# better62/MM-VQA-Healthcare

Measured on AMD Instinct MI355X. Metric: image-question pairs/sec, M3AE-base fine-tune step (fwd+bwd+AdamW) @384px, higher is better.
Workload: dtype bf16

## Files before the change

### include/m3ae_hip.h

```cpp
#ifndef M3AE_HIP_H
#define M3AE_HIP_H

#include <stdint.h>

#ifdef __cplusplus
extern "C" {
#endif

#define M3AE_ABI_VERSION 4

enum { M3AE_F32 = 0, M3AE_BF16 = 1 };
enum { M3AE_ACT_NONE = 0, M3AE_ACT_GELU = 1, M3AE_ACT_QUICKGELU = 2, M3AE_ACT_TANH = 3, M3AE_ACT_RELU = 4,
       M3AE_ACT_MULAUX = 5  };
enum { M3AE_ERR_ARG = -1, M3AE_ERR_UNSUPPORTED = -2, M3AE_ERR_ALIGN = -3, M3AE_ERR_WORKSPACE = -4 };

int m3ae_abi_version(void);
void m3ae_desc_sizes(int64_t out3[3]);
const char* m3ae_last_gemm_path(void);

typedef struct {
    int64_t M, N, K;
    int64_t batch1, batch2;
    const void* A; int64_t a_sm, a_sk, a_sb1, a_sb2;
    const void* B; int64_t b_sk, b_sn, b_sb1, b_sb2;
    void* C;       int64_t c_sm, c_sn, c_sb1, c_sb2;
    int32_t dtype_a, dtype_b, dtype_c;
    float alpha;
    int32_t accumulate;
    const float* bias;
    int32_t act;
    void* preact;
    const void* residual;
    const void* dact_aux;
    int32_t dact;
    int32_t force_generic;
    float* a_rowsum;
    float dropout_p;
    uint64_t dropout_seed;
    int32_t preact_grad;
    int32_t launch_flags;
    const void* dropout_salt;
} m3ae_gemm_desc;
enum { M3AE_GEMM_NO_PERSISTENT = 1 };
#define M3AE_GEMM_NT_VARIANT(v) ((((v) + 1) & 0xf) << 8)
#define M3AE_GEMM_TN_VARIANT(v) ((((v) + 1) & 0xf) << 12)
#define M3AE_GEMM_COL_GROUP(g) (((g) & 0xf) << 16)
int m3ae_gemm(const m3ae_gemm_desc* d, void* stream);

typedef struct {
    int64_t B, H, Lq, Lk, Dh;
    const void* q; int64_t q_sb, q_sl;
    const void* k; int64_t k_sb, k_sl;
    const void* v; int64_t v_sb, v_sl;
    void* o;       int64_t o_sb, o_sl;
    const float* key_mask;
    const float* pos_bias;
    float scale;
    int32_t causal;
    float* lse; int64_t lse_stride;
    int32_t dtype;
    void* workspace; int64_t workspace_bytes;
    const void* d_o;
    void* dq; void* dk; void* dv;
    float* delta;
    float* d_pos_bias;
    float dropout_p;
    uint64_t dropout_seed;
    const void* dropout_salt;
    int32_t launch_flags;
} m3ae_attn_desc;
enum { M3AE_ATTN_LEGACY_KERNELS = 1 };
int64_t m3ae_attn_workspace_bytes(const m3ae_attn_desc* d, int backward);
int m3ae_attn_fwd(const m3ae_attn_desc* d, void* stream);
int m3ae_attn_bwd(const m3ae_attn_desc* d, void* stream);
int m3ae_attn_probs(const m3ae_attn_desc* d, float* probs, int64_t p_sb, int64_t p_sh, int64_t p_sq, void* stream);

typedef struct {
    int32_t dir;
    int64_t B, Lq, Lk, D, H;
    const void* x;
    const void* y;
    const float* key_mask;
    const void *wq, *wq_t, *wkv, *wkv_t, *wo, *wo_t;
    const float *bq, *bkv, *bo, *ln_g, *ln_b;
    float ln_eps;
    float dropout_p;
    uint64_t seed_attn, seed_hidden;
    void* proj;
    void* prime;
    float* colbias;
    void* probs;
    void* probs_drop;
    float* rowsum;
    void* zctx;
    void* ctx;
    void* s;
    void* out;
    float *mean, *rstd;
    const void* d_out;
    void* dx;
    void* dy;
    float *g_wq, *g_wkv, *g_wo, *g_bq, *g_bkv, *g_bo, *g_ln_g, *g_ln_b;
    void* ws_ds;
    void* ws_dsd;
    void* ws_dscores;
    void* ws_dprime;
    void* ws_dproj;
    void* ws_dz;
    void* ws_dctx;
    float* ws_vec;
    float* ws_ln;
    int32_t launch_flags;
    const void* dropout_salt;
} m3ae_xattn_desc;
enum { M3AE_XATTN_NO_PERSISTENT = 1,
       M3AE_XATTN_LEGACY_CHAIN = 2     };
int m3ae_xattn_supported(const m3ae_xattn_desc* d);
int m3ae_xattn_bwd_supported(const m3ae_xattn_desc* d);
int64_t m3ae_xattn_probs_ld(const m3ae_xattn_desc* d);
int m3ae_xattn_fwd(const m3ae_xattn_desc* d, void* stream);
int m3ae_xattn_bwd(const m3ae_xattn_desc* d, void* stream);
int m3ae_xattn_probs_export(const m3ae_xattn_desc* d, int dropped, float* out, int64_t o_sb, int64_t o_sh, int64_t o_sq,
                            void* stream);

int m3ae_layernorm_fwd(const void* x, const float* gamma, const float* beta, void* y, float* mean, float* rstd,
                       int64_t M, int64_t D, float eps, int dtype, int act, int rms, void* stream);
int64_t m3ae_layernorm_bwd_blocks(int64_t M);
int m3ae_layernorm_bwd(const void* dy, const void* x, const float* gamma, const float* beta, const float* mean,
                       const float* rstd, void* dx, const void* dx_add, float* dgamma, float* dbeta, float* workspace,
                       int64_t M, int64_t D, int dtype, int act, int rms, void* stream);
int m3ae_layernorm_bwd_drop(const void* dy, const void* x, const float* gamma, const float* beta, const float* mean,
                            const float* rstd, void* dx, void* dx_drop, float dropout_p, uint64_t dropout_seed,
                            const void* dropout_salt, float* dgamma, float* dbeta, float* workspace, int64_t M, int64_t D,
                            int dtype, void* stream);
int m3ae_dropout(const void* x, void* out, uint8_t* keep_mask, int64_t rows, int64_t cols, float p, uint64_t seed,
                 const void* salt, int dtype, void* stream);

int m3ae_colsum(const void* x, float* out, int64_t M, int64_t N, int64_t ldx, int dtype, int accumulate,
                void* stream);

int m3ae_roberta_embed_fwd(const int64_t* ids, const float* word, const float* pos, const float* type, void* out,
                           int64_t B, int64_t S, int64_t D, int64_t pad_id, int dtype, void* stream);
int m3ae_roberta_embed_bwd(const int64_t* ids, const void* d_out, float* d_word, float* d_pos, float* d_type,
                           int64_t B, int64_t S, int64_t D, int64_t pad_id, int dtype, void* stream);

int m3ae_patchify(const float* img, void* out, int64_t B, int64_t R, int64_t P, int dtype, void* stream);
int m3ae_image_normalize_u8(const uint8_t* in, float* out, int64_t B, int64_t H, int64_t W, const float* mean3,
                            const float* std3, void* stream);
int m3ae_vit_tokens_fwd(const void* patch, const float* cls, const float* pos, void* out, int64_t B, int64_t G,
                        int64_t D, int dtype, void* stream);
int m3ae_vit_tokens_bwd(const void* d_out, void* d_patch, float* d_cls, float* d_pos, int64_t B, int64_t G,
                        int64_t D, int dtype, void* stream);

int m3ae_bce_logits(const void* logits, const float* targets, float* loss, void* d_logits, int64_t B, int64_t C,
// ... 36 lines not shown
```

### mm-vqa-healthcare_amd/csrc/attention.hip

```cpp
#include "common.h"
#include <stdlib.h>
#include <type_traits>

int m3ae_gemm_generic(const m3ae_gemm_desc& d, hipStream_t s);

namespace {

constexpr float LOG2E = 1.4426950408889634f;
constexpr int VRS = 192;
constexpr int TILE_LDS = 32 * VRS;

struct AttnArgs {
    const bf16_t* q; int64_t q_sb, q_sl;
    const bf16_t* k; int64_t k_sb, k_sl;
    const bf16_t* v; int64_t v_sb, v_sl;
    bf16_t* o; int64_t o_sb, o_sl;
    const float* key_mask;
    const float* pos_bias;
    float scale, scale_log2;
    int causal;
    float* lse; int64_t lse_stride;
    int64_t B, H, Lq, Lk;
    const bf16_t* d_o;
    bf16_t* dq; bf16_t* dk; bf16_t* dv;
// ... 214 lines not shown
    float m[NQ], l[NQ];
#pragma unroll
    for (int n = 0; n < NQ; ++n) {
        qi[n] = q0 + 32 * n + r;
        const int64_t qrow = qi[n] < a.Lq ? qi[n] : a.Lq - 1;
        const bf16_t* qp = a.q + b * a.q_sb + qrow * a.q_sl + head * 64;
#pragma unroll
        for (int ks = 0; ks < 4; ++ks) qf[n][ks] = row_frag(qp, ks, h);
        brow[n] = BIAS ? a.pos_bias + ((int64_t)head * a.Lq + qrow) * a.Lk : nullptr;
        o[n][0] = zero16(); o[n][1] = zero16();
        m[n] = -1e30f; l[n] = 0.f;
    }
    const bf16_t* kbase = a.k + b * a.k_sb + head * 64;
    const bf16_t* vbase = a.v + b * a.v_sb + head * 64;
    const float* mrow = MASK ? a.key_mask + b * a.Lk : nullptr;
    const int nkt = (int)((a.Lk + 31) / 32);

    s16x8 kreg = coop_load(kbase, a.k_sl, 0, a.Lk, t);
    s16x8 vreg = coop_load(vbase, a.v_sl, 0, a.Lk, t);
    put_row_img(lds, kreg, t);
    put_tr_img(lds + RIMG, vreg, t);
    if (nkt > 1) {
        kreg = coop_load(kbase, a.k_sl, 32, a.Lk, t);
        vreg = coop_load(vbase, a.v_sl, 32, a.Lk, t);
    }
    coop_barrier();
    for (int kt = 0; kt < nkt; ++kt) {
        const bool last = kt + 1 == nkt;
        s16x8 kreg2 = kreg, vreg2 = vreg;
        if (kt + 2 < nkt) {
            kreg2 = coop_load(kbase, a.k_sl, (int64_t)(kt + 2) * 32, a.Lk, t);
            vreg2 = coop_load(vbase, a.v_sl, (int64_t)(kt + 2) * 32, a.Lk, t);
        }
        const char* kimg = lds + (kt & 1) * BUF;
        const char* vimg = kimg + RIMG;
        if (active) {
            s16x8 kf[4], vf[4];
#pragma unroll
            for (int ks = 0; ks < 4; ++ks) { kf[ks] = get_row_frag(kimg, r, ks, h); vf[ks] = get_row_frag(vimg, r, ks, h); }
            f32x16 s[NQ];
#pragma unroll
            for (int n = 0; n < NQ; ++n) {
                s[n] = zero16();
#pragma unroll
                for (int ks = 0; ks < 4; ++ks) s[n] = mfma32(kf[ks], qf[n][ks], s[n]);
            }
            const int64_t key0 = (int64_t)kt * 32;
#pragma unroll
            for (int n = 0; n < NQ; ++n) {
                const uint64_t drow = (uint64_t)(((b * a.H + head) * a.Lq + qi[n]) * drop_ldk(a.Lk));
                if (last) score_to_prob<MASK, BIAS, CAUSAL, true, DROP>(s[n], m[n], l[n], o[n][0], o[n][1], a, mrow, brow[n], key0, qi[n], h, drow);
                else score_to_prob<MASK, BIAS, CAUSAL, false, DROP>(s[n], m[n], l[n], o[n][0], o[n][1], a, mrow, brow[n], key0, qi[n], h, drow);
            }
#pragma unroll
            for (int ss = 0; ss < 2; ++ss) {
                const s16x8 v0 = tr_frag(vimg, 0, ss, lane), v1 = tr_frag(vimg, 1, ss, lane);
#pragma unroll
                for (int n = 0; n < NQ; ++n) {
                    const s16x8 pb = pack_acc(s[n], ss);
                    o[n][0] = mfma32(v0, pb, o[n][0]);
                    o[n][1] = mfma32(v1, pb, o[n][1]);
                }
            }
        }
        if (!last) {
            char* nb = lds + ((kt + 1) & 1) * BUF;
            put_row_img(nb, kreg, t);
            put_tr_img(nb + RIMG, vreg, t);
        }
        kreg = kreg2; vreg = vreg2;
        coop_barrier();
    }
    if (!active) return;
#pragma unroll
    for (int n = 0; n < NQ; ++n) {
        const float ltot = l[n] + __shfl_xor(l[n], 32, 64);
        if (qi[n] < a.Lq) {
            store_rows(a.o + b * a.o_sb + qi[n] * a.o_sl + head * 64, o[n][0], o[n][1], 1.0f / ltot, h);
            if (h == 0) a.lse[(b * a.H + head) * a.lse_stride + qi[n]] = m[n] + log2f(ltot);
        } else if (h == 0 && qi[n] < a.lse_stride) {
            a.lse[(b * a.H + head) * a.lse_stride + qi[n]] = 0.f;
        }
    }
}

template <bool MASK, bool DROP>
__global__ __launch_bounds__(256, 2) void attn_probs_kernel(AttnArgs a, float* __restrict__ P, int64_t p_sb, int64_t p_sh,
                                                             int64_t p_sq) {
    if (DROP) drop_resolve(a.drop);
    __shared__ __attribute__((aligned(16))) char lds[2 * RIMG];
    const int t = threadIdx.x;
    const int lane = t & 63;
    const int wave = __builtin_amdgcn_readfirstlane(t >> 6);
    const int r = lane & 31, h = lane >> 5;
    const AttnBlock blk = attn_block();
    const int head = blk.head;
    const int64_t b = blk.b;
    const int64_t q0 = ((int64_t)blk.bx * 4 + wave) * 32;
    const bool active = q0 < a.Lq;

    const int64_t qa = q0 + r < a.Lq ? q0 + r : a.Lq - 1;
    const bf16_t* qp = a.q + b * a.q_sb + qa * a.q_sl + head * 64;
    s16x8 qf[4];
#pragma unroll
    for (int ks = 0; ks < 4; ++ks) qf[ks] = row_frag(qp, ks, h);
    const float* lrow = a.lse + (b * a.H + head) * a.lse_stride;
    float nl[16];
#pragma unroll
    for (int reg = 0; reg < 16; ++reg) {
        const int64_t q = q0 + crow(reg, h);
        nl[reg] = -lrow[q < a.Lq ? q : a.Lq - 1];
    }
    float* prow = P + b * p_sb + head * p_sh;
    const uint64_t drow0 = (uint64_t)((b * a.H + head) * a.Lq) * drop_ldk(a.Lk);
    const bf16_t* kbase = a.k + b * a.k_sb + head * 64;
    const float* mrow = MASK ? a.key_mask + b * a.Lk : nullptr;
    const int nkt = (int)((a.Lk + 31) / 32);

    s16x8 kreg = coop_load(kbase, a.k_sl, 0, a.Lk, t);
    put_row_img(lds, kreg, t);
    if (nkt > 1) kreg = coop_load(kbase, a.k_sl, 32, a.Lk, t);
    coop_barrier();
    for (int kt = 0; kt < nkt; ++kt) {
        const bool last = kt + 1 == nkt;
        s16x8 kreg2 = kreg;
        if (kt + 2 < nkt) kreg2 = coop_load(kbase, a.k_sl, (int64_t)(kt + 2) * 32, a.Lk, t);
        const char* kimg = lds + (kt & 1) * RIMG;
        if (active) {
            f32x16 s = zero16();
#pragma unroll
            for (int ks = 0; ks < 4; ++ks) s = mfma32(qf[ks], get_row_frag(kimg, r, ks, h), s);
            const int64_t key = (int64_t)kt * 32 + r;
            const bool kin = key < a.Lk;
            const float madd = MASK ? mrow[kin ? key : a.Lk - 1] * LOG2E : 0.f;
#pragma unroll
            for (int reg = 0; reg < 16; ++reg) {
                const int64_t q = q0 + crow(reg, h);
                float p = fast_exp2(fmaf(s[reg], a.scale_log2, madd) + nl[reg]);
                if (DROP) p = drop_keep(a.drop, drow0 + (uint64_t)q * drop_ldk(a.Lk) + (uint64_t)key) ? p * a.drop.inv_keep : 0.f;
                if (kin && q < a.Lq) prow[q * p_sq + key] = p;
            }
        }
        if (!last) put_row_img(lds + ((kt + 1) & 1) * RIMG, kreg, t);
        kreg = kreg2;
        coop_barrier();
    }
}

template <bool MASK, bool BIAS, bool CAUSAL, bool DROP>
__global__ __launch_bounds__(256, 2) void attn_bwd_dq_coop_kernel(AttnArgs a) {
    if (DROP) drop_resolve(a.drop);
    constexpr int BUF = RIMG + TILE_LDS + RIMG;
    __shared__ __attribute__((aligned(16))) char lds[2 * BUF];
    const int t = threadIdx.x;
    const int lane = t & 63;
    const int wave = __builtin_amdgcn_readfirstlane(t >> 6);
    const int r = lane & 31, h = lane >> 5;
    const AttnBlock blk = attn_block();
    const int head = blk.head;
    const int64_t b = blk.b;
    const int64_t q0 = ((int64_t)blk.bx * 4 + wave) * 32;
    const bool active = q0 < a.Lq;

    const int64_t qi = q0 + r;
    const int64_t qrow = qi < a.Lq ? qi : a.Lq - 1;
    const bf16_t* qp = a.q + b * a.q_sb + qrow * a.q_sl + head * 64;
// ... 610 lines not shown
    dot = wave_sum(dot);
    for (int64_t j = lane; j < Lk; j += 64) d[j] = p[j] * (d[j] - dot);
}

__global__ void pos_bias_grad_kernel(const float* dS, float* dpb, int64_t B, int64_t HQK) {
    const int64_t i = (int64_t)blockIdx.x * blockDim.x + threadIdx.x;
    if (i >= HQK) return;
    float acc = 0.f;
    for (int64_t b = 0; b < B; ++b) acc += dS[b * HQK + i];
    dpb[i] += acc;
}

m3ae_gemm_desc bgemm(const m3ae_attn_desc& d) {
    m3ae_gemm_desc g{};
    g.batch1 = d.B; g.batch2 = d.H;
    g.dtype_a = g.dtype_b = g.dtype_c = M3AE_F32;
    g.alpha = 1.0f;
    return g;
}

int attn_f32_scores(const m3ae_attn_desc& d, float* S, hipStream_t s) {
    const int64_t QK = d.Lq * d.Lk;
    m3ae_gemm_desc g = bgemm(d);
    g.M = d.Lq; g.N = d.Lk; g.K = d.Dh; g.alpha = d.scale;
    g.A = d.q; g.a_sm = d.q_sl; g.a_sk = 1; g.a_sb1 = d.q_sb; g.a_sb2 = d.Dh;
    g.B = d.k; g.b_sk = 1; g.b_sn = d.k_sl; g.b_sb1 = d.k_sb; g.b_sb2 = d.Dh;
    g.C = S; g.c_sm = d.Lk; g.c_sn = 1; g.c_sb1 = d.H * QK; g.c_sb2 = QK;
    int rc = m3ae_gemm_generic(g, s);
    if (rc) return rc;
    const int64_t rows = d.B * d.H * d.Lq;
    hipLaunchKernelGGL(softmax_rows_kernel, dim3((unsigned)cdiv(rows, 4)), dim3(256), 0, s, S, d.key_mask, d.pos_bias,
                       d.B, d.H, d.Lq, d.Lk, d.causal);
    return hip_launch_status();
}

AttnArgs to_args(const m3ae_attn_desc& d) {
    AttnArgs a{};
    a.q = (const bf16_t*)d.q; a.q_sb = d.q_sb; a.q_sl = d.q_sl;
    a.k = (const bf16_t*)d.k; a.k_sb = d.k_sb; a.k_sl = d.k_sl;
    a.v = (const bf16_t*)d.v; a.v_sb = d.v_sb; a.v_sl = d.v_sl;
    a.o = (bf16_t*)d.o; a.o_sb = d.o_sb; a.o_sl = d.o_sl;
    a.key_mask = d.key_mask; a.pos_bias = d.pos_bias;
    a.scale = d.scale; a.scale_log2 = d.scale * LOG2E; a.causal = d.causal;
    a.lse = d.lse; a.lse_stride = d.lse_stride;
    a.B = d.B; a.H = d.H; a.Lq = d.Lq; a.Lk = d.Lk;
    a.d_o = (const bf16_t*)d.d_o; a.dq = (bf16_t*)d.dq; a.dk = (bf16_t*)d.dk; a.dv = (bf16_t*)d.dv;
    a.delta = d.delta; a.d_pos_bias = d.d_pos_bias;
    a.has_drop = d.dropout_p > 0.f;
    a.drop = make_drop(d.dropout_p, d.dropout_seed, d.dropout_salt);
    return a;
}

bool bf16_layout_ok(const m3ae_attn_desc& d, bool bwd) {
    auto al = [](const void* p) { return (((uintptr_t)p) & 15) == 0; };
    auto st = [](int64_t x) { return x % 8 == 0; };
    bool ok = d.Dh == 64 && al(d.q) && al(d.k) && al(d.v) && al(d.o) && st(d.q_sl) && st(d.k_sl) && st(d.v_sl) &&
              st(d.o_sl) && st(d.q_sb) && st(d.k_sb) && st(d.v_sb) && st(d.o_sb) && d.lse && d.lse_stride >= d.Lq &&
              d.lse_stride % 32 == 0;
    if (bwd) ok = ok && al(d.d_o) && al(d.dq) && al(d.dk) && al(d.dv) && d.delta;
    return ok;
}

}


extern "C" int64_t m3ae_attn_workspace_bytes(const m3ae_attn_desc* d, int backward) {
    if (!d) return 0;
    if (d->dtype == M3AE_BF16) return 0;
    const int64_t one = d->B * d->H * d->Lq * d->Lk * (int64_t)sizeof(float);
    return backward ? 2 * one : one;
}

extern "C" int m3ae_attn_fwd(const m3ae_attn_desc* dp, void* stream) {
    if (!dp || !dp->q || !dp->k || !dp->v || !dp->o) return M3AE_ERR_ARG;
    const m3ae_attn_desc& d = *dp;
    if (d.B <= 0 || d.H <= 0 || d.Lq <= 0 || d.Lk <= 0 || d.Dh <= 0) return M3AE_ERR_ARG;
    hipStream_t s = (hipStream_t)stream;
    if (d.dtype == M3AE_BF16) {
        if (!bf16_layout_ok(d, false)) return M3AE_ERR_UNSUPPORTED;
        if (d.H > 65535 || d.B > 65535) return M3AE_ERR_UNSUPPORTED;
        AttnArgs a = to_args(d);
        int rc = 0;
        dim3 grid((unsigned)cdiv(d.Lq, 128), (unsigned)d.H, (unsigned)d.B);
        ATTN_DISPATCH_COOP(rc, attn_fwd_coop_kernel, grid, s, a, 1, );
        if (rc) return rc;
        return hip_launch_status();
    }
    if (d.dtype != M3AE_F32) return M3AE_ERR_UNSUPPORTED;
    if (!d.workspace || d.workspace_bytes < m3ae_attn_workspace_bytes(dp, 0)) return M3AE_ERR_WORKSPACE;
    float* S = (float*)d.workspace;
    int rc = attn_f32_scores(d, S, s);
    if (rc) return rc;
    if (d.dropout_p > 0.f &&
        (rc = m3ae_dropout(S, S, nullptr, d.B * d.H * d.Lq, d.Lk, d.dropout_p, d.dropout_seed, d.dropout_salt, M3AE_F32, stream)))
        return rc;
    const int64_t QK = d.Lq * d.Lk;
    m3ae_gemm_desc g = bgemm(d);
    g.M = d.Lq; g.N = d.Dh; g.K = d.Lk;
    g.A = S; g.a_sm = d.Lk; g.a_sk = 1; g.a_sb1 = d.H * QK; g.a_sb2 = QK;
    g.B = d.v; g.b_sk = d.v_sl; g.b_sn = 1; g.b_sb1 = d.v_sb; g.b_sb2 = d.Dh;
    g.C = d.o; g.c_sm = d.o_sl; g.c_sn = 1; g.c_sb1 = d.o_sb; g.c_sb2 = d.Dh;
    return m3ae_gemm_generic(g, s);
}

extern "C" int m3ae_attn_probs(const m3ae_attn_desc* dp, float* probs, int64_t p_sb, int64_t p_sh, int64_t p_sq, void* stream) {
    if (!dp || !dp->q || !dp->k || !probs) return M3AE_ERR_ARG;
    const m3ae_attn_desc& d = *dp;
    if (d.B <= 0 || d.H <= 0 || d.Lq <= 0 || d.Lk <= 0 || d.Dh <= 0) return M3AE_ERR_ARG;
    if (p_sq < d.Lk || p_sh <= 0 || p_sb <= 0) return M3AE_ERR_ARG;
    if (d.pos_bias || d.causal) return M3AE_ERR_UNSUPPORTED;
    hipStream_t s = (hipStream_t)stream;
    if (d.dtype == M3AE_BF16) {
        auto al = [](const void* p) { return (((uintptr_t)p) & 15) == 0; };
        auto st = [](int64_t x) { return x % 8 == 0; };
        if (d.Dh != 64 || !al(d.q) || !al(d.k) || !st(d.q_sl) || !st(d.k_sl) || !st(d.q_sb) || !st(d.k_sb) || !d.lse ||
            d.lse_stride < d.Lq || d.lse_stride % 32 != 0)
            return M3AE_ERR_UNSUPPORTED;
        if (d.H > 65535 || d.B > 65535) return M3AE_ERR_UNSUPPORTED;
        AttnArgs a = to_args(d);
        dim3 grid((unsigned)cdiv(d.Lq, 128), (unsigned)d.H, (unsigned)d.B);
        if (a.key_mask) {
            if (a.has_drop) hipLaunchKernelGGL((attn_probs_kernel<true, true>), grid, dim3(256), 0, s, a, probs, p_sb, p_sh, p_sq);
            else hipLaunchKernelGGL((attn_probs_kernel<true, false>), grid, dim3(256), 0, s, a, probs, p_sb, p_sh, p_sq);
        } else {
            if (a.has_drop) hipLaunchKernelGGL((attn_probs_kernel<false, true>), grid, dim3(256), 0, s, a, probs, p_sb, p_sh, p_sq);
            else hipLaunchKernelGGL((attn_probs_kernel<false, false>), grid, dim3(256), 0, s, a, probs, p_sb, p_sh, p_sq);
        }
        return hip_launch_status();
    }
    if (d.dtype != M3AE_F32) return M3AE_ERR_UNSUPPORTED;
    if (p_sq != d.Lk || p_sh != d.Lq * d.Lk || p_sb != d.H * d.Lq * d.Lk) return M3AE_ERR_UNSUPPORTED;
    int rc = attn_f32_scores(d, probs, s);
    if (rc) return rc;
    if (d.dropout_p > 0.f)
        return m3ae_dropout(probs, probs, nullptr, d.B * d.H * d.Lq, d.Lk, d.dropout_p, d.dropout_seed, d.dropout_salt, M3AE_F32, stream);
    return 0;
}

extern "C" int m3ae_attn_bwd(const m3ae_attn_desc* dp, void* stream) {
    if (!dp || !dp->q || !dp->k || !dp->v || !dp->o || !dp->d_o || !dp->dq || !dp->dk || !dp->dv)
        return M3AE_ERR_ARG;
    const m3ae_attn_desc& d = *dp;
    hipStream_t s = (hipStream_t)stream;
    if (d.dtype == M3AE_BF16) {
        if (!bf16_layout_ok(d, true)) return M3AE_ERR_UNSUPPORTED;
        AttnArgs a = to_args(d);
        dim3 gq((unsigned)cdiv(cdiv(d.Lq, 32), 4), (unsigned)d.H, (unsigned)d.B);
        dim3 gk((unsigned)cdiv(cdiv(d.Lk, 32), 4), (unsigned)d.H, (unsigned)d.B);
        int rc = 0;
        const bool gen4 = !a.pos_bias && !a.causal && !(d.launch_flags & M3AE_ATTN_LEGACY_KERNELS);
        if (gen4) {
            if (a.key_mask) { if (a.has_drop) hipLaunchKernelGGL((attn_bwd_dq2_kernel<true, true, 2>), gq, dim3(256), 0, s, a);
                              else hipLaunchKernelGGL((attn_bwd_dq2_kernel<true, false, TPS_PLAIN>), gq, dim3(256), 0, s, a); }
            else { if (a.has_drop) hipLaunchKernelGGL((attn_bwd_dq2_kernel<false, true, 2>), gq, dim3(256), 0, s, a);
                   else hipLaunchKernelGGL((attn_bwd_dq2_kernel<false, false, TPS_PLAIN>), gq, dim3(256), 0, s, a); }
        } else {
            ATTN_DISPATCH_COOP(rc, attn_bwd_dq_coop_kernel, gq, s, a, );
        }
        if (gen4) {
            if (a.key_mask) { if (a.has_drop) hipLaunchKernelGGL((attn_bwd_dkdv2_kernel<true, true, 2>), gk, dim3(256), 0, s, a);
                              else hipLaunchKernelGGL((attn_bwd_dkdv2_kernel<true, false, TPS_PLAIN>), gk, dim3(256), 0, s, a); }
            else { if (a.has_drop) hipLaunchKernelGGL((attn_bwd_dkdv2_kernel<false, true, 2>), gk, dim3(256), 0, s, a);
                   else hipLaunchKernelGGL((attn_bwd_dkdv2_kernel<false, false, TPS_PLAIN>), gk, dim3(256), 0, s, a); }
        } else {
            ATTN_DISPATCH_COOP(rc, attn_bwd_dkdv_coop_kernel, gk, s, a, );
        }
// ... 52 lines not shown
```

### mm-vqa-healthcare_amd/m3ae_amd/_lib.py

```python
import ctypes as C
import os

_PKG = os.path.dirname(os.path.abspath(__file__))
DIAGNOSTIC = os.environ.get("M3AE_DIAGNOSTIC_LIB", "") == "1"
LIB_PATH = os.path.join(_PKG, "lib_diag" if DIAGNOSTIC else "lib", "libm3ae_hip.so")

F32, BF16 = 0, 1
ACT_NONE, ACT_GELU, ACT_QUICKGELU, ACT_TANH, ACT_RELU, ACT_MULAUX = 0, 1, 2, 3, 4, 5

vp, i64, i32, f32 = C.c_void_p, C.c_int64, C.c_int32, C.c_float


class GemmDesc(C.Structure):
    _fields_ = [
        ("M", i64), ("N", i64), ("K", i64), ("batch1", i64), ("batch2", i64),
        ("A", vp), ("a_sm", i64), ("a_sk", i64), ("a_sb1", i64), ("a_sb2", i64),
        ("B", vp), ("b_sk", i64), ("b_sn", i64), ("b_sb1", i64), ("b_sb2", i64),
        ("C", vp), ("c_sm", i64), ("c_sn", i64), ("c_sb1", i64), ("c_sb2", i64),
        ("dtype_a", i32), ("dtype_b", i32), ("dtype_c", i32),
        ("alpha", f32), ("accumulate", i32), ("bias", vp), ("act", i32), ("preact", vp), ("residual", vp),
        ("dact_aux", vp), ("dact", i32), ("force_generic", i32), ("a_rowsum", vp),
        ("dropout_p", f32), ("dropout_seed", C.c_uint64), ("preact_grad", i32), ("launch_flags", i32), ("dropout_salt", vp),
    ]


class AttnDesc(C.Structure):
    _fields_ = [
        ("B", i64), ("H", i64), ("Lq", i64), ("Lk", i64), ("Dh", i64),
        ("q", vp), ("q_sb", i64), ("q_sl", i64),
        ("k", vp), ("k_sb", i64), ("k_sl", i64),
        ("v", vp), ("v_sb", i64), ("v_sl", i64),
        ("o", vp), ("o_sb", i64), ("o_sl", i64),
        ("key_mask", vp), ("pos_bias", vp), ("scale", f32), ("causal", i32),
        ("lse", vp), ("lse_stride", i64), ("dtype", i32), ("workspace", vp), ("workspace_bytes", i64),
        ("d_o", vp), ("dq", vp), ("dk", vp), ("dv", vp), ("delta", vp), ("d_pos_bias", vp),
        ("dropout_p", f32), ("dropout_seed", C.c_uint64), ("dropout_salt", vp), ("launch_flags", i32),
    ]


class XattnDesc(C.Structure):
    _fields_ = [
        ("dir", i32), ("B", i64), ("Lq", i64), ("Lk", i64), ("D", i64), ("H", i64),
        ("x", vp), ("y", vp), ("key_mask", vp),
        ("wq", vp), ("wq_t", vp), ("wkv", vp), ("wkv_t", vp), ("wo", vp), ("wo_t", vp),
        ("bq", vp), ("bkv", vp), ("bo", vp), ("ln_g", vp), ("ln_b", vp),
        ("ln_eps", f32), ("dropout_p", f32), ("seed_attn", C.c_uint64), ("seed_hidden", C.c_uint64),
        ("proj", vp), ("prime", vp), ("colbias", vp), ("probs", vp), ("probs_drop", vp), ("rowsum", vp),
        ("zctx", vp), ("ctx", vp), ("s", vp), ("out", vp), ("mean", vp), ("rstd", vp),
        ("d_out", vp), ("dx", vp), ("dy", vp),
        ("g_wq", vp), ("g_wkv", vp), ("g_wo", vp), ("g_bq", vp), ("g_bkv", vp), ("g_bo", vp), ("g_ln_g", vp), ("g_ln_b", vp),
        ("ws_ds", vp), ("ws_dsd", vp), ("ws_dscores", vp), ("ws_dprime", vp), ("ws_dproj", vp), ("ws_dz", vp), ("ws_dctx", vp),
        ("ws_vec", vp), ("ws_ln", vp), ("launch_flags", i32), ("dropout_salt", vp),
    ]


GEMM_NO_PERSISTENT = 1
ATTN_LEGACY_KERNELS = 1
XATTN_NO_PERSISTENT, XATTN_LEGACY_CHAIN = 1, 2
ABI_VERSION = 4


_SIGS = {
    "m3ae_abi_version": (C.c_int, []),
    "m3ae_desc_sizes": (None, [C.POINTER(i64)]),
    "m3ae_last_gemm_path": (C.c_char_p, []),
    "m3ae_gemm": (C.c_int, [C.POINTER(GemmDesc), vp]),
    "m3ae_attn_workspace_bytes": (i64, [C.POINTER(AttnDesc), C.c_int]),
    "m3ae_attn_fwd": (C.c_int, [C.POINTER(AttnDesc), vp]),
    "m3ae_attn_bwd": (C.c_int, [C.POINTER(AttnDesc), vp]),
    "m3ae_attn_probs": (C.c_int, [C.POINTER(AttnDesc), vp, i64, i64, i64, vp]),
    "m3ae_xattn_supported": (C.c_int, [C.POINTER(XattnDesc)]),
    "m3ae_xattn_bwd_supported": (C.c_int, [C.POINTER(XattnDesc)]),
    "m3ae_xattn_probs_ld": (i64, [C.POINTER(XattnDesc)]),
    "m3ae_xattn_fwd": (C.c_int, [C.POINTER(XattnDesc), vp]),
    "m3ae_xattn_bwd": (C.c_int, [C.POINTER(XattnDesc), vp]),
    "m3ae_xattn_probs_export": (C.c_int, [C.POINTER(XattnDesc), C.c_int, vp, i64, i64, i64, vp]),
    "m3ae_layernorm_fwd": (C.c_int, [vp, vp, vp, vp, vp, vp, i64, i64, f32, C.c_int, C.c_int, C.c_int, vp]),
    "m3ae_layernorm_bwd_blocks": (i64, [i64]),
    "m3ae_layernorm_bwd": (C.c_int, [vp, vp, vp, vp, vp, vp, vp, vp, vp, vp, vp, i64, i64, C.c_int, C.c_int, C.c_int, vp]),
    "m3ae_layernorm_bwd_drop": (C.c_int, [vp, vp, vp, vp, vp, vp, vp, vp, f32, C.c_uint64, vp, vp, vp, vp, i64, i64, C.c_int, vp]),
    "m3ae_dropout": (C.c_int, [vp, vp, vp, i64, i64, f32, C.c_uint64, vp, C.c_int, vp]),
    "m3ae_colsum": (C.c_int, [vp, vp, i64, i64, i64, C.c_int, C.c_int, vp]),
    "m3ae_roberta_embed_fwd": (C.c_int, [vp, vp, vp, vp, vp, i64, i64, i64, i64, C.c_int, vp]),
    "m3ae_roberta_embed_bwd": (C.c_int, [vp, vp, vp, vp, vp, i64, i64, i64, i64, C.c_int, vp]),
    "m3ae_patchify": (C.c_int, [vp, vp, i64, i64, i64, C.c_int, vp]),
    "m3ae_image_normalize_u8": (C.c_int, [vp, vp, i64, i64, i64, C.POINTER(C.c_float), C.POINTER(C.c_float), vp]),
    "m3ae_vit_tokens_fwd": (C.c_int, [vp, vp, vp, vp, i64, i64, i64, C.c_int, vp]),
    "m3ae_vit_tokens_bwd": (C.c_int, [vp, vp, vp, vp, i64, i64, i64, C.c_int, vp]),
    "m3ae_bce_logits": (C.c_int, [vp, vp, vp, vp, i64, i64, f32, C.c_int, vp]),
    "m3ae_xent": (C.c_int, [vp, vp, vp, vp, vp, i64, i64, i64, f32, C.c_int, vp]),
    "m3ae_adamw": (C.c_int, [vp, vp, vp, vp, vp, i64, f32, f32, f32, f32, f32, i64, f32, vp, vp]),
    "m3ae_cast_transpose": (C.c_int, [vp, vp, vp, i64, i64, vp]),
    "m3ae_cast_transpose_batched": (C.c_int, [vp, C.c_int, i64, vp]),
    "m3ae_transpose_bf16_batched": (C.c_int, [vp, C.c_int, i64, vp]),
    "m3ae_cast": (C.c_int, [vp, vp, i64, C.c_int, C.c_int, vp]),
    "m3ae_zero": (C.c_int, [vp, i64, vp]),
    "m3ae_add": (C.c_int, [vp, vp, vp, i64, C.c_int, vp]),
    "m3ae_act_fwd": (C.c_int, [vp, vp, i64, C.c_int, C.c_int, vp]),
    "m3ae_act_bwd": (C.c_int, [vp, vp, vp, i64, C.c_int, C.c_int, vp]),
    "m3ae_gather_rows": (C.c_int, [vp, vp, vp, i64, i64, C.c_int, vp]),
    "m3ae_scatter_add_rows": (C.c_int, [vp, vp, vp, i64, i64, C.c_int, vp]),
    "m3ae_mask_ranks": (C.c_int, [vp, vp, vp, vp, i64, i64, i64, vp]),
    "m3ae_mim_targets": (C.c_int, [vp, vp, i64, i64, i64, i64, i64, C.c_int, vp]),
    "m3ae_mim_loss_fwd": (C.c_int, [vp, vp, vp, vp, vp, i64, i64, i64, C.c_int, vp]),
    "m3ae_mim_loss_bwd": (C.c_int, [vp, vp, vp, vp, vp, vp, i64, i64, i64, C.c_int, vp]),
    "m3ae_selftest": (C.c_int, [vp, vp]),
}

EXPORTS = tuple(_SIGS)
_lib = None


class M3AEHipError(RuntimeError):
    pass


def lib():
    global _lib
    if _lib is None:
        if not os.path.exists(LIB_PATH):
            raise M3AEHipError(f"{LIB_PATH} is missing: build it with `python -m m3ae_amd.build` "
                               f"(or __graft_entry__.build()); this package has no CPU fallback")
        import torch
        if DIAGNOSTIC:
            import warnings
            warnings.warn(f"m3ae_amd: loading the DIAGNOSTIC library {LIB_PATH} (timing-only builds may compute wrong results)")
        l = C.CDLL(LIB_PATH)
        for name, (res, args) in _SIGS.items():
            fn = getattr(l, name)
            fn.restype, fn.argtypes = res, args
        if l.m3ae_abi_version() != ABI_VERSION:
            raise M3AEHipError(f"ABI version mismatch: library {l.m3ae_abi_version()}, binding {ABI_VERSION}")
        sizes = (i64 * 3)()
        l.m3ae_desc_sizes(sizes)
        mine = (C.sizeof(GemmDesc), C.sizeof(AttnDesc), C.sizeof(XattnDesc))
        if tuple(sizes) != mine:
            raise M3AEHipError(f"descriptor layout mismatch: library {tuple(sizes)}, binding {mine}")
        _lib = l
    return _lib

# ... 7 lines not shown
```

### mm-vqa-healthcare_amd/m3ae_amd/ops.py

```python
import ctypes as C
import math
import os

import torch

from . import _lib
from ._lib import (ACT_GELU, ACT_MULAUX, ACT_NONE, ACT_QUICKGELU, ACT_RELU, ACT_TANH, BF16, F32, AttnDesc, GemmDesc, XattnDesc,
                   check)

grad_ready_hook = None
SAVE_DACT = os.environ.get("M3AE_SAVE_DACT", "1") != "0"
NT_NO_PERSISTENT = os.environ.get("M3AE_NT_NO_PERSISTENT", "0") == "1"
GEMM_NT_VARIANT, GEMM_TN_VARIANT, GEMM_COL_GROUP = int(os.environ.get("M3AE_GEMM_NT_VARIANT", -1)), int(os.environ.get("M3AE_GEMM_TN_VARIANT", -1)), int(os.environ.get("M3AE_GEMM_COL_GROUP", 0))


ATTN_LEGACY = os.environ.get("M3AE_ATTN_LEGACY", "0") == "1"
GEMM_ST_POLICY = int(os.environ.get("M3AE_GEMM_ST_POLICY", 0))


def _gemm_flags():
    return ((1 if NT_NO_PERSISTENT else 0) | (((GEMM_NT_VARIANT + 1) & 0xF) << 8) | (((GEMM_TN_VARIANT + 1) & 0xF) << 12)
            | ((GEMM_COL_GROUP & 0xF) << 16) | ((GEMM_ST_POLICY & 0x3) << 20))
PROFILE = None


def _prof_begin():
    if PROFILE is None:
        return None
    e0 = torch.cuda.Event(enable_timing=True)
    e0.record()
    return e0


def _prof_end(e0, kind, dims):
    if e0 is None:
        return
    e1 = torch.cuda.Event(enable_timing=True)
    e1.record()
    PROFILE.append((kind, dims, e0, e1))


_drop_base, _drop_ctr = 0x5EED, 0


def set_dropout_seed(seed):
    global _drop_base, _drop_ctr
    _drop_base, _drop_ctr = int(seed) & 0xFFFFFFFF, 0


DROPOUT_SALT = None


def _salt():
    return None if DROPOUT_SALT is None else C.c_void_p(DROPOUT_SALT.data_ptr())


def next_dropout_seed():
    global _drop_ctr
    _drop_ctr += 1
    return ((_drop_base << 32) | (_drop_ctr & 0xFFFFFFFF)) & 0xFFFFFFFFFFFFFFFF


def _dt(t):
    if t.dtype == torch.float32:
        return F32
    if t.dtype == torch.bfloat16:
        return BF16
    raise TypeError(f"unsupported dtype {t.dtype}")


_raw_stream = getattr(torch._C, "_cuda_getCurrentRawStream", None)
_dev_index = None


def _stream():
    global _dev_index
    if _raw_stream is None:
        return C.c_void_p(torch.cuda.current_stream().cuda_stream)
    if _dev_index is None:
        _dev_index = torch.cuda.current_device()
    return C.c_void_p(_raw_stream(_dev_index))


def _p(t):
    return None if t is None else C.c_void_p(t.data_ptr())


def _need_cuda(t):
    if not t.is_cuda:
        raise _lib.M3AEHipError("m3ae_amd ops run on the GPU only (no CPU fallback); got a CPU tensor")
    if _dev_index is not None and t.device.index != _dev_index:
        raise _lib.M3AEHipError(f"m3ae_amd ops were first used on cuda:{_dev_index}; got a tensor on {t.device} "
                                f"(one process drives one GPU: call torch.cuda.set_device before the first op)")


def compute_weight(w):
    return getattr(w, "m3ae_c", w)


# ... 296 lines not shown
        y = torch.empty_like(xc)
        mean = torch.empty(M, dtype=torch.float32, device=x.device)
        rstd = torch.empty(M, dtype=torch.float32, device=x.device)
        check(_lib.lib().m3ae_layernorm_fwd(_p(xc), _p(gamma), _p(beta), _p(y), _p(mean), _p(rstd), M, D, eps, _dt(xc),
                                            act, int(rms), _stream()), "m3ae_layernorm_fwd")
        ctx.save_for_backward(xc, mean, rstd)
        ctx.gamma, ctx.beta, ctx.act, ctx.rms = gamma, beta, act, rms
        return y

    @staticmethod
    def backward(ctx, dy):
        xc, mean, rstd = ctx.saved_tensors
        D = xc.shape[-1]
        M = xc.numel() // D
        dyc = dy.contiguous()
        dx = torch.empty_like(xc)
        L = _lib.lib()
        nblk = L.m3ae_layernorm_bwd_blocks(M)
        ws = torch.empty(2 * nblk * D, dtype=torch.float32, device=xc.device)
        gg = _grad_buf(ctx.gamma)
        gb = _grad_buf(ctx.beta) if ctx.beta is not None else None
        check(L.m3ae_layernorm_bwd(_p(dyc), _p(xc), _p(ctx.gamma), _p(ctx.beta), _p(mean), _p(rstd), _p(dx), None,
                                   _p(gg), _p(gb), _p(ws), M, D, _dt(xc), ctx.act, int(ctx.rms), _stream()),
              "m3ae_layernorm_bwd")
        _done(ctx.gamma)
        _done(ctx.beta)
        return dx, None, None, None, None, None


def layer_norm(x, gamma, beta, eps, act=ACT_NONE, rms=False):
    return LayerNormFn.apply(x, gamma, beta, eps, act, rms)


def ln_fwd_raw(x2, ln, act=ACT_NONE, rms=False):
    M, D = x2.shape
    y = torch.empty_like(x2)
    mean = None if rms else torch.empty(M, dtype=torch.float32, device=x2.device)
    rstd = torch.empty(M, dtype=torch.float32, device=x2.device)
    check(_lib.lib().m3ae_layernorm_fwd(_p(x2), _p(ln.weight), _p(ln.bias), _p(y), _p(mean), _p(rstd), M, D, ln.eps,
                                        _dt(x2), act, int(rms), _stream()), "m3ae_layernorm_fwd")
    return y, mean, rstd


def ln_bwd_raw(dy, x2, ln, mean, rstd, dx_add=None, act=ACT_NONE, rms=False, drop=None):
    M, D = x2.shape
    L = _lib.lib()
    dx = torch.empty_like(x2)
    nblk = L.m3ae_layernorm_bwd_blocks(M)
    ws = torch.empty(2 * nblk * D, dtype=torch.float32, device=x2.device)
    train = ln.weight.requires_grad
    gg = _grad_buf(ln.weight) if train else None
    gb = _grad_buf(ln.bias) if (train and ln.bias is not None) else None
    if drop is not None and drop[0] > 0:
        assert dx_add is None and act == ACT_NONE and not rms
        dxd = torch.empty_like(x2)
        check(L.m3ae_layernorm_bwd_drop(_p(dy), _p(x2), _p(ln.weight), _p(ln.bias), _p(mean), _p(rstd), _p(dx), _p(dxd),
                                        drop[0], drop[1], _salt(), _p(gg), _p(gb), _p(ws), M, D, _dt(x2), _stream()),
              "m3ae_layernorm_bwd_drop")
        if train:
            _done(ln.weight)
            _done(ln.bias)
        return dx, dxd
    check(L.m3ae_layernorm_bwd(_p(dy), _p(x2), _p(ln.weight), _p(ln.bias), _p(mean), _p(rstd), _p(dx), _p(dx_add),
                               _p(gg), _p(gb), _p(ws), M, D, _dt(x2), act, int(rms), _stream()), "m3ae_layernorm_bwd")
    if train:
        _done(ln.weight)
        _done(ln.bias)
    return dx


def _attn_desc(B, H, Lq, Lk, Dh, q, k, v, o, key_mask, pos_bias, scale, causal, lse, lse_stride, dtype):
    d = AttnDesc()
    d.B, d.H, d.Lq, d.Lk, d.Dh = B, H, Lq, Lk, Dh
    d.q, d.q_sb, d.q_sl = q.data_ptr(), q.stride(0), q.stride(1)
    d.k, d.k_sb, d.k_sl = k.data_ptr(), k.stride(0), k.stride(1)
    d.v, d.v_sb, d.v_sl = v.data_ptr(), v.stride(0), v.stride(1)
    d.o, d.o_sb, d.o_sl = o.data_ptr(), o.stride(0), o.stride(1)
    d.key_mask = key_mask.data_ptr() if key_mask is not None else None
    d.pos_bias = pos_bias.data_ptr() if pos_bias is not None else None
    d.scale, d.causal = scale, int(causal)
    d.lse = lse.data_ptr() if lse is not None else None
    d.lse_stride = lse_stride
    d.dtype = dtype
    d.launch_flags = _lib.ATTN_LEGACY_KERNELS if ATTN_LEGACY else 0
    return d


def _attn_ws(d, backward, device):
    n = _lib.lib().m3ae_attn_workspace_bytes(C.byref(d), int(backward))
    if n <= 0:
        return None
    ws = torch.empty(n, dtype=torch.uint8, device=device)
    d.workspace, d.workspace_bytes = ws.data_ptr(), n
    return ws


def attn_forward(q, k, v, heads, key_mask=None, pos_bias=None, scale=None, causal=False, dropout=None):
    _need_cuda(q)
    B, Lq, D = q.shape
    Lk = k.shape[1]
    Dh = D // heads
    if q.dtype == torch.bfloat16 and Dh != 64:
        o32, lse = attn_forward(q.float(), k.float(), v.float(), heads, key_mask, pos_bias, scale, causal, dropout)
        return o32.to(torch.bfloat16), lse
    scale = (1.0 / math.sqrt(Dh)) if scale is None else scale
    o = torch.empty((B, Lq, D), dtype=q.dtype, device=q.device)
    lse_stride = (Lq + 31) // 32 * 32
    lse = (torch.empty if q.dtype == torch.bfloat16 else torch.zeros)((B, heads, lse_stride), dtype=torch.float32, device=q.device)
    d = _attn_desc(B, heads, Lq, Lk, Dh, q, k, v, o, key_mask, pos_bias, scale, causal, lse, lse_stride, _dt(q))
    if dropout is not None and dropout[0] > 0:
        d.dropout_p, d.dropout_seed = dropout
        d.dropout_salt = _salt()
    ws = _attn_ws(d, False, q.device)
    e0 = _prof_begin()
    check(_lib.lib().m3ae_attn_fwd(C.byref(d), _stream()), "m3ae_attn_fwd")
    _prof_end(e0, "attn_fwd", (B, heads, Lq, Lk, Dh))
    del ws
    return o, lse


def attn_backward(q, k, v, o, lse, do, dq, dk, dv, heads, key_mask=None, pos_bias=None, scale=None, causal=False,
                  d_pos_bias=None, dropout=None):
    B, Lq, D = q.shape
    Lk = k.shape[1]
    Dh = D // heads
    if q.dtype == torch.bfloat16 and Dh != 64:
        f = [t.float() for t in (q, k, v, o, do)]
        g = [torch.empty_like(t) for t in f[:3]]
        attn_backward(f[0], f[1], f[2], f[3].contiguous(), lse, f[4].contiguous(), g[0], g[1], g[2], heads, key_mask,
                      pos_bias, scale, causal, d_pos_bias, dropout)
        for dst, src in zip((dq, dk, dv), g):
            dst.copy_(src)
        return
    scale = (1.0 / math.sqrt(Dh)) if scale is None else scale
    assert do.stride() == o.stride() and dq.stride() == q.stride() and dk.stride() == k.stride() and dv.stride() == v.stride()
    d = _attn_desc(B, heads, Lq, Lk, Dh, q, k, v, o, key_mask, pos_bias, scale, causal, lse, lse.shape[-1], _dt(q))
    delta = torch.empty_like(lse) if q.dtype == torch.bfloat16 else torch.zeros_like(lse)
    d.d_o, d.dq, d.dk, d.dv, d.delta = do.data_ptr(), dq.data_ptr(), dk.data_ptr(), dv.data_ptr(), delta.data_ptr()
    d.d_pos_bias = d_pos_bias.data_ptr() if d_pos_bias is not None else None
    if dropout is not None and dropout[0] > 0:
        d.dropout_p, d.dropout_seed = dropout
        d.dropout_salt = _salt()
    ws = _attn_ws(d, True, q.device)
    e0 = _prof_begin()
    check(_lib.lib().m3ae_attn_bwd(C.byref(d), _stream()), "m3ae_attn_bwd")
    _prof_end(e0, "attn_bwd", (B, heads, Lq, Lk, Dh))
    del ws, delta


def attn_probs(q, k, lse, heads, key_mask=None, scale=None, dropout=None):
    _need_cuda(q)
    B, Lq, D = q.shape
    Lk = k.shape[1]
    Dh = D // heads
    if q.dtype == torch.bfloat16 and Dh != 64:
        return attn_probs(q.float(), k.float(), None, heads, key_mask, scale, dropout)
    scale = (1.0 / math.sqrt(Dh)) if scale is None else scale
    out = torch.empty((B, heads, Lq, Lk), dtype=torch.float32, device=q.device)
    lse_stride = lse.shape[-1] if lse is not None else 0
    d = _attn_desc(B, heads, Lq, Lk, Dh, q, k, k, q, key_mask, None, scale, False, lse, lse_stride, _dt(q))
    if dropout is not None and dropout[0] > 0:
        d.dropout_p, d.dropout_seed = dropout
        d.dropout_salt = _salt()
    e0 = _prof_begin()
    check(_lib.lib().m3ae_attn_probs(C.byref(d), C.c_void_p(out.data_ptr()), out.stride(0), out.stride(1), out.stride(2),
                                     _stream()), "m3ae_attn_probs")
    _prof_end(e0, "attn_probs", (B, heads, Lq, Lk, Dh))
# ... 884 lines not shown
```

Baseline: 1361.

## Add double-buffered attention forward kernel with scalar path for odd tail rows

Adds a new attention forward kernel for Dh=64 without position bias or causal masking, used when Lq and Lk are multiples of 32 or one more (for example 577 tokens at 384px with a CLS token). Key and value tiles are prefetched two steps ahead into registers and double-buffered in LDS, so global loads overlap MFMA compute. The single leftover key is handled up front with a scalar dot product, and the single leftover query row goes through a per-row FMA path instead of padded MFMA tiles. The aim is to cut load stalls and wasted work on partial tiles in the existing cooperative kernel, at the cost of more code and a separate edge-case path. An environment flag restores the old kernel.

```diff
diff --git a/include/m3ae_hip.h b/include/m3ae_hip.h
--- a/include/m3ae_hip.h
+++ b/include/m3ae_hip.h
@@ -69,7 +69,7 @@
     const void* dropout_salt;
     int32_t launch_flags;
 } m3ae_attn_desc;
-enum { M3AE_ATTN_LEGACY_KERNELS = 1 };
+enum { M3AE_ATTN_LEGACY_KERNELS = 1, M3AE_ATTN_LEGACY_FWD = 2 };
 int64_t m3ae_attn_workspace_bytes(const m3ae_attn_desc* d, int backward);
 int m3ae_attn_fwd(const m3ae_attn_desc* d, void* stream);
 int m3ae_attn_bwd(const m3ae_attn_desc* d, void* stream);
diff --git a/mm-vqa-healthcare_amd/csrc/attention.hip b/mm-vqa-healthcare_amd/csrc/attention.hip
--- a/mm-vqa-healthcare_amd/csrc/attention.hip
+++ b/mm-vqa-healthcare_amd/csrc/attention.hip
@@ -320,6 +320,193 @@
             a.lse[(b * a.H + head) * a.lse_stride + qi[n]] = 0.f;
         }
     }
+}
+
+DEVINL float bf_lo(uint32_t w) { return __uint_as_float(w << 16); }
+DEVINL float bf_hi(uint32_t w) { return __uint_as_float(w & 0xffff0000u); }
+DEVINL float dot64(const s16x8 (&x)[4], const s16x8 (&y)[4]) {
+    float acc0 = 0.f, acc1 = 0.f;
+#pragma unroll
+    for (int ks = 0; ks < 4; ++ks) {
+        u32x4 u = __builtin_bit_cast(u32x4, x[ks]);
+        const u32x4 w = __builtin_bit_cast(u32x4, y[ks]);
+        asm volatile("" : "+v"(u));
+#pragma unroll
+        for (int i = 0; i < 4; ++i) {
+            acc0 = fmaf(bf_lo(u[i]), bf_lo(w[i]), acc0);
+            acc1 = fmaf(bf_hi(u[i]), bf_hi(w[i]), acc1);
+        }
+    }
+    return acc0 + acc1;
+}
+
+#ifndef M3AE_G5_DROP_BLOCKS
+#define M3AE_G5_DROP_BLOCKS 4
+#endif
+template <bool MASK, bool DROP>
+__global__ __launch_bounds__(256, (MASK && DROP) ? 2 : DROP ? M3AE_G5_DROP_BLOCKS : 4) void attn_fwd_g5_kernel(AttnArgs a) {
+    if (DROP) drop_resolve(a.drop);
+    constexpr int BUF = RIMG + TILE_LDS;
+    __shared__ __attribute__((aligned(16))) char lds[2 * BUF];
+    __shared__ __attribute__((aligned(16))) float prow[32];
+    const int t = threadIdx.x;
+    const int lane = t & 63;
+    const int wave = __builtin_amdgcn_readfirstlane(t >> 6);
+    const int r = lane & 31, h = lane >> 5;
+    const AttnBlock blk = attn_block();
+    const int head = blk.head;
+    const int64_t b = blk.b;
+    const int64_t q0 = ((int64_t)blk.bx * 4 + wave) * 32;
+    const bool full = q0 + 32 <= a.Lq;
+    const bool rowq = !full && q0 < a.Lq;
+    const int nfk = (int)(a.Lk >> 5);
+
+    const int64_t qi = full ? q0 + r : q0;
+    const int64_t qc = qi < a.Lq ? qi : a.Lq - 1;
+    s16x8 qf[4];
+    {
+        const bf16_t* qp = a.q + b * a.q_sb + qc * a.q_sl + head * 64;
+#pragma unroll
+        for (int ks = 0; ks < 4; ++ks) qf[ks] = row_frag(qp, ks, h);
+    }
+    const bf16_t* kbase = a.k + b * a.k_sb + head * 64;
+    const bf16_t* vbase = a.v + b * a.v_sb + head * 64;
+    const float* mrow = MASK ? a.key_mask + b * a.Lk : nullptr;
+    const uint64_t drow = (uint64_t)(((b * a.H + head) * a.Lq + qc) * drop_ldk(a.Lk));
+
+    s16x8 kreg = coop_load(kbase, a.k_sl, 0, a.Lk, t);
+    s16x8 vreg = coop_load(vbase, a.v_sl, 0, a.Lk, t);
+
+    auto run = [&](auto row_tag) {
+        constexpr bool ROW = decltype(row_tag)::value;
+        f32x16 o0 = zero16(), o1 = zero16();
+        float m = -1e30f, l = 0.f, ox0 = 0.f, ox1 = 0.f;
+        if (a.Lk & 31) {
+            const int64_t kr = (int64_t)nfk * 32;
+            const bf16_t* kp = kbase + kr * a.k_sl;
+            s16x8 kf[4];
+#pragma unroll
+            for (int ks = 0; ks < 4; ++ks) kf[ks] = row_frag(kp, ks, h);
+            float x = dot64(qf, kf);
+            x = (x + __shfl_xor(x, 32, 64)) * a.scale_log2;
+            if (MASK) x = fmaf(mrow[kr], LOG2E, x);
+            m = x;
+            float p = 1.f;
+            if (DROP) p = drop_keep(a.drop, drow + (uint64_t)kr) ? a.drop.inv_keep : 0.f;
+            const bf16_t* vp = vbase + kr * a.v_sl;
+            if (!ROW) {
+                l = h == 0 ? 1.f : 0.f;
+#pragma unroll
+                for (int g4 = 0; g4 < 4; ++g4) {
+                    const u32x2 w0 = *(const u32x2*)(vp + 8 * g4 + 4 * h), w1 = *(const u32x2*)(vp + 32 + 8 * g4 + 4 * h);
+                    o0[4 * g4 + 0] = p * bf_lo(w0[0]); o0[4 * g4 + 1] = p * bf_hi(w0[0]);
+                    o0[4 * g4 + 2] = p * bf_lo(w0[1]); o0[4 * g4 + 3] = p * bf_hi(w0[1]);
+                    o1[4 * g4 + 0] = p * bf_lo(w1[0]); o1[4 * g4 + 1] = p * bf_hi(w1[0]);
+                    o1[4 * g4 + 2] = p * bf_lo(w1[1]); o1[4 * g4 + 3] = p * bf_hi(w1[1]);
+                }
+            } else {
+                l = r == 0 ? 1.f : 0.f;
+                if (h == 0) { ox0 = p * bf2f(vp[r]); ox1 = p * bf2f(vp[32 + r]); }
+            }
+        }
+
+        put_row_img(lds, kreg, t);
+        put_tr_img(lds + RIMG, vreg, t);
+        if (nfk > 1) {
+            kreg = coop_load(kbase, a.k_sl, 32, a.Lk, t);
+            vreg = coop_load(vbase, a.v_sl, 32, a.Lk, t);
+        }
+        coop_barrier();
+        for (int kt = 0; kt < nfk; ++kt) {
+            s16x8 kreg2 = kreg, vreg2 = vreg;
+            if (kt + 2 < nfk) {
+                kreg2 = coop_load(kbase, a.k_sl, (int64_t)(kt + 2) * 32, a.Lk, t);
+                vreg2 = coop_load(vbase, a.v_sl, (int64_t)(kt + 2) * 32, a.Lk, t);
+            }
+            const char* kimg = lds + (kt & 1) * BUF;
+            const char* vimg = kimg + RIMG;
+            const int64_t key0 = (int64_t)kt * 32;
+            if (!ROW && full) {
+                s16x8 kf[4];
+#pragma unroll
+                for (int ks = 0; ks < 4; ++ks) kf[ks] = get_row_frag(kimg, r, ks, h);
+                f32x16 s = zero16();
+#pragma unroll
+                for (int ks = 0; ks < 4; ++ks) s = mfma32(kf[ks], qf[ks], s);
+                score_to_prob<MASK, false, false, false, DROP>(s, m, l, o0, o1, a, mrow, nullptr, key0, qi, h, drow);
+#pragma unroll
+                for (int ss = 0; ss < 2; ++ss) {
+                    const s16x8 v0 = tr_frag(vimg, 0, ss, lane), v1 = tr_frag(vimg, 1, ss, lane);
+                    const s16x8 pb = pack_acc(s, ss);
+                    o0 = mfma32(v0, pb, o0);
+                    o1 = mfma32(v1, pb, o1);
+                }
+            } else if (ROW) {
+                s16x8 kf[4];
+#pragma unroll
+                for (int ks = 0; ks < 4; ++ks) kf[ks] = get_row_frag(kimg, r, ks, h);
+                float x = dot64(qf, kf);
+                x = (x + __shfl_xor(x, 32, 64)) * a.scale_log2;
+                if (MASK) x = fmaf(mrow[key0 + r], LOG2E, x);
+                float tmax = x;
+#pragma unroll
+                for (int o = 16; o > 0; o >>= 1) tmax = fmaxf(tmax, __shfl_xor(tmax, o, 64));
+                if (tmax > m) {
+                    const float alpha = fast_exp2(m - tmax);
+                    m = tmax;
+                    l *= alpha; ox0 *= alpha; ox1 *= alpha;
+                }
+                float p = fast_exp2(x - m);
+                l += p;
+                if (DROP) p = drop_keep(a.drop, drow + (uint64_t)(key0 + r)) ? p * a.drop.inv_keep : 0.f;
+                if (h == 0) prow[r] = p;
+                asm volatile("" ::: "memory");
+                f32x4 pk[4];
+#pragma unroll
+                for (int g = 0; g < 4; ++g) pk[g] = *(const f32x4*)(prow + 8 * g + 4 * h);
+#pragma unroll
+                for (int ss = 0; ss < 2; ++ss) {
+                    const u32x4 v0 = __builtin_bit_cast(u32x4, tr_frag(vimg, 0, ss, lane));
+                    const u32x4 v1 = __builtin_bit_cast(u32x4, tr_frag(vimg, 1, ss, lane));
+#pragma unroll
+                    for (int j2 = 0; j2 < 4; ++j2) {
+                        const float p0 = pk[2 * ss + (j2 >> 1)][2 * (j2 & 1)], p1 = pk[2 * ss + (j2 >> 1)][2 * (j2 & 1) + 1];
+                        ox0 = fmaf(p0, bf_lo(v0[j2]), ox0); ox0 = fmaf(p1, bf_hi(v0[j2]), ox0);
+                        ox1 = fmaf(p0, bf_lo(v1[j2]), ox1); ox1 = fmaf(p1, bf_hi(v1[j2]), ox1);
+                    }
+                }
+                asm volatile("" ::: "memory");
+            }
+            if (kt + 1 < nfk) {
+                char* nb = lds + ((kt + 1) & 1) * BUF;
+                put_row_img(nb, kreg, t);
+                put_tr_img(nb + RIMG, vreg, t);
+            }
+            kreg = kreg2; vreg = vreg2;
+            coop_barrier();
+        }
+        float* lse = a.lse + (b * a.H + head) * a.lse_stride;
+        if (!ROW && full) {
+            const float ltot = l + __shfl_xor(l, 32, 64);
+            store_rows(a.o + b * a.o_sb + qi * a.o_sl + head * 64, o0, o1, 1.0f / ltot, h);
+            if (h == 0) lse[qi] = m + log2f(ltot);
+        } else if (ROW) {
+            ox0 += __shfl_xor(ox0, 32, 64);
+            ox1 += __shfl_xor(ox1, 32, 64);
+            float ltot = l;
+#pragma unroll
+            for (int o = 16; o > 0; o >>= 1) ltot += __shfl_xor(ltot, o, 64);
+            if (h == 0) {
+                const float inv = 1.0f / ltot;
+                bf16_t* op = a.o + b * a.o_sb + q0 * a.o_sl + head * 64;
+                op[r] = f2bf(ox0 * inv);
+                op[32 + r] = f2bf(ox1 * inv);
+                if (q0 + r < a.lse_stride) lse[q0 + r] = r == 0 ? m + log2f(ltot) : 0.f;
+            }
+        }
+    };
+    if (rowq) run(std::true_type{});
+    else run(std::false_type{});
 }
 
 template <bool MASK, bool DROP>
@@ -1096,6 +1283,18 @@
         AttnArgs a = to_args(d);
         int rc = 0;
         dim3 grid((unsigned)cdiv(d.Lq, 128), (unsigned)d.H, (unsigned)d.B);
+        const bool g5 = !a.pos_bias && !a.causal && d.Lk >= 32 && (d.Lk & 31) <= 1 && (d.Lq & 31) <= 1 &&
+                        !(d.launch_flags & M3AE_ATTN_LEGACY_FWD);
+        if (g5) {
+            if (a.key_mask) {
+                if (a.has_drop) hipLaunchKernelGGL((attn_fwd_g5_kernel<true, true>), grid, dim3(256), 0, s, a);
+                else hipLaunchKernelGGL((attn_fwd_g5_kernel<true, false>), grid, dim3(256), 0, s, a);
+            } else {
+                if (a.has_drop) hipLaunchKernelGGL((attn_fwd_g5_kernel<false, true>), grid, dim3(256), 0, s, a);
+                else hipLaunchKernelGGL((attn_fwd_g5_kernel<false, false>), grid, dim3(256), 0, s, a);
+            }
+            return hip_launch_status();
+        }
         ATTN_DISPATCH_COOP(rc, attn_fwd_coop_kernel, grid, s, a, 1, );
         if (rc) return rc;
         return hip_launch_status();
diff --git a/mm-vqa-healthcare_amd/m3ae_amd/_lib.py b/mm-vqa-healthcare_amd/m3ae_amd/_lib.py
--- a/mm-vqa-healthcare_amd/m3ae_amd/_lib.py
+++ b/mm-vqa-healthcare_amd/m3ae_amd/_lib.py
@@ -55,7 +55,7 @@
 
 
 GEMM_NO_PERSISTENT = 1
-ATTN_LEGACY_KERNELS = 1
+ATTN_LEGACY_KERNELS, ATTN_LEGACY_FWD = 1, 2
 XATTN_NO_PERSISTENT, XATTN_LEGACY_CHAIN = 1, 2
 ABI_VERSION = 4
 
diff --git a/mm-vqa-healthcare_amd/m3ae_amd/ops.py b/mm-vqa-healthcare_amd/m3ae_amd/ops.py
--- a/mm-vqa-healthcare_amd/m3ae_amd/ops.py
+++ b/mm-vqa-healthcare_amd/m3ae_amd/ops.py
@@ -15,6 +15,7 @@
 
 
 ATTN_LEGACY = os.environ.get("M3AE_ATTN_LEGACY", "0") == "1"
+ATTN_LEGACY_FWD = os.environ.get("M3AE_ATTN_LEGACY_FWD", "0") == "1"
 GEMM_ST_POLICY = int(os.environ.get("M3AE_GEMM_ST_POLICY", 0))
 
 
@@ -477,7 +478,7 @@
     d.lse = lse.data_ptr() if lse is not None else None
     d.lse_stride = lse_stride
     d.dtype = dtype
-    d.launch_flags = _lib.ATTN_LEGACY_KERNELS if ATTN_LEGACY else 0
+    d.launch_flags = (_lib.ATTN_LEGACY_KERNELS if ATTN_LEGACY else 0) | (_lib.ATTN_LEGACY_FWD if ATTN_LEGACY_FWD else 0)
     return d
 
 
```

After: 1364 (median of 5 runs). Within noise of the previous version (+0.2%).
